# cafferychen777/flashdeconv

Measured on AMD Instinct MI355X. Metric: spots/sec to convergence (1M x 2000 x 30), higher is better.
Workload: dtype f64; 1 GPU; 1000000 spots x 2000 genes x 30 types, sketch_dim 512, k_neighbors 6, gaussian/raw family, Y float32 in HBM, tol 1e-4, max_iter 100; converged=True

## Files before the change

### flashdeconv_amd/_lib.py

```python
import ctypes
import os
import threading

import numpy as np

_HERE = os.path.dirname(os.path.abspath(__file__))
LIB_PATH = os.path.join(_HERE, "libfdx.so")

c_int = ctypes.c_int
c_i32 = ctypes.c_int32
c_i64 = ctypes.c_int64
c_double = ctypes.c_double
c_void_p = ctypes.c_void_p
c_size_t = ctypes.c_size_t
p_double = ctypes.POINTER(ctypes.c_double)
p_i64 = ctypes.POINTER(ctypes.c_int64)
p_i32 = ctypes.POINTER(ctypes.c_int32)


class FdxError(RuntimeError):
    """A libfdx call failed (message from fdx_last_error())."""


class SolveInfo(ctypes.Structure):
# ... 199 lines not shown
    "fdx_comm_init_local": (c_int, [c_void_p, c_i32, ctypes.POINTER(c_void_p)]),
    "fdx_comm_init_loopback": (c_int, [c_i32, c_i32, ctypes.POINTER(c_void_p)]),
    "fdx_comm_destroy": (c_int, [c_void_p]),
    "fdx_comm_info": (c_int, [c_void_p, p_i32, p_i32]),
    "fdx_comm_rccl_count": (c_int, [c_void_p, p_i32]),
    "fdx_comm_allreduce_sum_dev": (c_int, [c_void_p, c_void_p, c_i32, c_void_p]),
    "fdx_sharded_solve_dev": (c_int, [c_void_p, c_void_p, c_void_p, c_i64, c_void_p, c_i32, c_double, c_double, c_double, c_i32,
                                      c_void_p, c_void_p, c_i64, ctypes.POINTER(SolveInfo), p_double, p_i32, c_void_p]),
    "fdx_solver_padded_k": (c_i32, [c_i32]),
    "fdx_shard_fit_dev": (c_int, [c_void_p, c_void_p, c_void_p, c_i32, c_i64, c_i32, c_i64, p_double, c_i32, p_i32, p_double, p_double,
                                  ctypes.POINTER(ShardFitParams), c_void_p, c_void_p, p_double, ctypes.POINTER(ShardFitInfo), c_void_p]),
    "fdx_sharded_solve_padded_dev": (c_int, [c_void_p, c_void_p, c_void_p, c_i64, c_void_p, c_i32, c_i32, c_double, c_double, c_double,
                                             c_i32, c_void_p, c_void_p, c_i64, ctypes.POINTER(SolveInfo), p_double, p_i32, c_void_p]),
    "fdx_tile_schedule": (c_int, [p_i32, p_double, c_i32, c_i32, c_i32, c_i32, c_i32, p_i32, p_i32, c_void_p, p_i32, p_double,
                                  c_void_p, c_i64]),
    "fdx_sketch_path": (c_int, [c_i32, c_void_p, c_i64, c_i32, c_i32, c_i32, c_i32, p_i32, p_double, p_i32, p_i32]),
    "fdx_column_sums": (c_int, [c_void_p, c_i32, c_i64, c_i32, p_double]),
    "fdx_log1p_f32": (c_int, [c_void_p, ctypes.c_float, c_i64, c_void_p]),
    "fdx_graph_build_knn": (c_int, [p_double, c_i64, c_i32, c_i32, ctypes.POINTER(c_void_p)]),
    "fdx_graph_build_radius": (c_int, [p_double, c_i64, c_i32, c_double, ctypes.POINTER(c_void_p)]),
    "fdx_nearest_distance": (c_int, [p_double, c_i64, c_i32, p_double]),
    "fdx_graph_export_csr": (c_int, [c_void_p, p_i64, p_i32]),
    "fdx_graph_from_csr": (c_int, [p_i64, p_i64, c_i64, ctypes.POINTER(c_void_p)]),
    "fdx_graph_destroy": (c_int, [c_void_p]),
    "fdx_graph_info": (c_int, [c_void_p, p_i64, p_i64, p_i32]),
    "fdx_graph_knn_ties": (c_int, [c_void_p, p_i64]),
    "fdx_graph_knn_far": (c_int, [c_void_p, ctypes.POINTER(c_i32)]),
    "fdx_kdtree_set_threads": (c_int, [c_i32]),
    "fdx_kdtree_tune": (c_int, [c_i32, c_i64]),
    "fdx_ckdtree_indices_dev": (c_int, [c_void_p, c_i64, c_i32, p_i64, p_i32, c_void_p]),
# ... 421 lines not shown
```

### flashdeconv_amd/csrc/tile_kernels.cpp

```cpp
#include "fdx_env.h"
#include <algorithm>
#include <cmath>
#include <cstdlib>
#include <memory>
#include <mutex>

#include "fdx_internal.h"
#include "fdx_kernels.h"
#include "sketch_plan.h"
#include "tile_device.h"
#include "tile_plan.h"
#include "tile_variant.h"

namespace fdx {

struct TilePlanDevice {
    TilePlanHost h;
    DevBuf w, off, len, ent_base, slot_bucket;
    int RS = 0;
    int WB = 0;
    size_t lds = 0;
};

const double* log_table_dev(hipStream_t st) {
    static std::mutex mu;
    static double* tabs[64] = {};
    int dev = 0;
    if (hipGetDevice(&dev) != hipSuccess || dev < 0 || dev >= 64) return nullptr;
    std::lock_guard<std::mutex> lock(mu);
    if (!tabs[dev]) {
        std::vector<double> t((size_t)LOG_TAB_N);
        for (int i = 0; i < LOG_TAB_N; ++i) {
            const unsigned bits = (unsigned)(LOG_TAB_BASE + i) << LOG_TAB_SHIFT;
            float c;
// ... 23 lines not shown
}

static bool tile_cfg(int dtype, int mode, int K, int d, int logv, TileVariant* out) {
    if ((dtype != FDX_F32 && dtype != FDX_F64) || K < 1 || K > 64 || d < 1) return false;
    if (mode != FDX_PRE_RAW && mode != FDX_PRE_LOG_CPM && mode != FDX_PRE_LOG_CPM_SPARSE) return false;
    const bool raw = mode == FDX_PRE_RAW;
    TileVariant v = raw ? TileVariant{12, 4, 11} : TileVariant{16, 0, 8};
    v.TT = (K + 15) / 16;
    if (K > 32 || d > 4 * v.NWC * v.JW) {
        v = raw ? TileVariant{12, 4, 22, 4, true} : TileVariant{8, 0, 32, 4, true};
        if (d > 4 * v.NWC * v.JW) return false;
    }
    v.logv = (dtype == FDX_F32 && !raw && logv != 0) ? 2 : 0;
    v.avl2 = v.wide || (!raw && v.logv == 0);
    v.wg = v.wide && raw;
    *out = v;
    return true;
}

static size_t tile_lds_bytes(int RS, int NE, int mode, int WB = 0) {
    const size_t NEp = ((size_t)NE + 7) & ~(size_t)7;
    const size_t below = 2 * ((size_t)WB + (size_t)TILE_ROWS * RS) + NEp * (WB ? 2 : 10) + 2 * TILE_ROWS * (8 + 4);
    if (mode == FDX_PRE_RAW) return below;
    return below <= (size_t)LOG_TAB_LDS ? (size_t)160 * 1024 : (size_t)161 * 1024;
}

static const TilePlanDevice* tile_plan_for(const SketchPlan& sp, int dtype, int mode, const TileVariant& v, hipStream_t st) {
    const int sz = dtype == FDX_F32 ? 4 : 8;
    const int key = ((dtype == FDX_F32 ? 0 : 1) * 2 + (mode != FDX_PRE_RAW ? 1 : 0)) * 3 + (v.wide ? 2 : v.TT - 1);
    static_assert(SketchPlan::kTileKeys == 12, "key space of the schedules: input type x raw / log x {one tile, two tiles, wide}");
    std::lock_guard<std::mutex> lock(sp.tile_mu);
    if (sp.tile_tried[key]) return sp.tile[key].get();
    sp.tile_tried[key] = true;
    const bool dbg = fdx::env("FDX_DEBUG") != nullptr;
    if (!sp.scatter_ok || sp.host_bucket.empty()) return nullptr;
    const size_t red_bytes = tile_red_bytes(v.NWC, v.avl2, v.TT);
    const int unit = (v.wide ? 128 : 1024) / sz;
    std::unique_ptr<TilePlanDevice> best;
    int GB0 = (int)round_up(sp.G, unit);
    while ((size_t)(v.wg ? round_up((GB0 + 1) * 8, 16) : 0) + (size_t)TILE_ROWS * (GB0 * sz + TILE_ROW_PAD) < red_bytes) GB0 += unit;
    for (int GB = GB0; GB >= unit; GB -= unit) {
        const int RS = GB * sz + TILE_ROW_PAD;
        const int WB = v.wg ? (int)round_up((GB + 1) * 8, 16) : 0;
        if ((size_t)WB + (size_t)TILE_ROWS * RS < red_bytes) break;
        if (tile_lds_bytes(RS, sp.G, mode, WB) > 160 * 1024) continue;
        auto cand = std::make_unique<TilePlanDevice>();
        if (!build_tile_plan(sp.host_bucket.data(), sp.host_w.data(), sp.G, sp.d, v.NWC, v.JW, GB, &cand->h)) return nullptr;
        cand->RS = RS;
        cand->WB = WB;
        cand->lds = tile_lds_bytes(RS, cand->h.NE, mode, WB);
        if (dbg) std::fprintf(stderr, "[fdx] tile plan: G=%d d=%d waves=%d+%d GB=%d blocks=%d NE=%d steps=%d lds=%zu\n", sp.G, sp.d, v.NWC,
                              v.NWL, GB, cand->h.NBLK, cand->h.NE, cand->h.steps, cand->lds);
        if (cand->lds > 160 * 1024) continue;
        best = std::move(cand);
        break;
    }
    if (!best) return nullptr;
    TilePlanDevice& t = *best;
    auto up = [&](DevBuf& b, const void* src, size_t bytes) -> int {
        FDX_TRY(b.alloc(bytes));
        FDX_TRY(copy_h2d(b.p, src, bytes, st));
        return 0;
    };
    const int jp = JW_PAD(v.JW);
    std::vector<unsigned char> len_pad((size_t)v.NWC * t.h.NBLK * jp + 16, 0);
    for (int wv = 0; wv < v.NWC; ++wv)
        for (int c = 0; c < t.h.NBLK; ++c)
            for (int j = 0; j < v.JW; ++j)
                len_pad[((size_t)wv * t.h.NBLK + c) * jp + j] = t.h.len[((size_t)wv * t.h.NBLK + c) * v.JW + j];
    std::vector<double> wg_tab;
    if (t.WB) {
        const int per = t.WB / 8;
        wg_tab.assign((size_t)t.h.NBLK * per, 0.0);
        for (int g = 0; g < sp.G; ++g)
            if (sp.host_bucket[(size_t)g] >= 0) wg_tab[(size_t)(g / t.h.GB) * per + g % t.h.GB] = sp.host_w[(size_t)g];
        for (size_t i = 0; i < t.h.off.size(); ++i)
            if (t.h.gene[i] < 0) t.h.off[i] = (unsigned short)t.h.GB;
    }
    if ((t.WB ? up(t.w, wg_tab.data(), wg_tab.size() * 8) : up(t.w, t.h.w.data(), t.h.w.size() * 8)) ||
        up(t.off, t.h.off.data(), t.h.off.size() * 2) || up(t.len, len_pad.data(), len_pad.size()) || up(t.ent_base, t.h.ent_base.data(), t.h.ent_base.size() * 4) ||
        up(t.slot_bucket, t.h.slot_bucket.data(), t.h.slot_bucket.size() * 4))
        return nullptr;
    if (hipStreamSynchronize(st) != hipSuccess) return nullptr;
    sp.tile[key] = std::move(best);
    return sp.tile[key].get();
}

__global__ void tile_xa_kernel(const double* __restrict__ Xs, const int* __restrict__ slot_bucket, int K, int d, int n_groups,
                               int TT, double* __restrict__ XA) {
    const int i = blockIdx.x * blockDim.x + threadIdx.x;
    if (i >= n_groups * TT * 64) return;
    const int lane = i & 63, t = (i >> 6) % TT, wj = (i >> 6) / TT;
// ... 17 lines not shown
                       const SketchPlanDev& plan, const double* Xs, int K, double* H, long long ldh, double* row_sumsq,
                       hipStream_t st) {
    if (n <= 0) return 0;
    TileVariant v;
    const TilePlanDevice* t = plan.owner && tile_cfg(dtype, mode, K, d, tile_logv(), &v) ? tile_plan_for(*plan.owner, dtype, mode, v, st) : nullptr;
    if (!t) return fail(FDX_ERR_INVALID, "tile sketch: no schedule for this shape");
    const void* kern = dtype == FDX_F32 ? tile_kernel<float>(mode, v) : tile_kernel<double>(mode, v);
    if (!kern) {
        char msg[128];
        std::snprintf(msg, sizeof msg, "tile sketch: no kernel for dtype %d mode %d, waves %d + %d x %d, TT %d, AVL2 %d, LOGV %d, WG %d",
                      dtype, mode, v.NWC, v.NWL, v.JW, v.TT, (int)v.avl2, v.logv, (int)v.wg);
        return fail(FDX_ERR_INVALID, msg);
    }
    TileArgs a{};
    a.ldy = ldy; a.n = n; a.ldh = ldh; a.G = G; a.d = d; a.K = K;
    a.NE = t->h.NE; a.GB = t->h.GB; a.NBLK = t->h.NBLK; a.RS = t->RS; a.jw_used = t->h.jw_used; a.WB = t->WB;
    const double* w_tab = t->w.as<double>();
    const unsigned short* off_tab = t->off.as<unsigned short>();
    const unsigned char* len_tab = t->len.as<unsigned char>();
    const int* ent_base = t->ent_base.as<int>();
    const int* slot_bucket = t->slot_bucket.as<int>();
    const double* log_tab = nullptr;
    if (mode != FDX_PRE_RAW) {
        log_tab = log_table_dev(st);
        if (!log_tab) return fail(FDX_ERR_HIP, "tile sketch: log table upload failed");
    }
    const long long n_tiles = (n + TILE_ROWS - 1) / TILE_ROWS;
    const int grid = (int)std::min<long long>(n_tiles, 256);
    DevBuf xa;
    const double* XA = nullptr;
    if (v.avl2) {
// ... 37 lines not shown
extern "C" int fdx_log1p_f32(const float* y, float scale, int64_t n, float* out) {
    using namespace fdx;
    FDX_REQUIRE(n >= 0 && (n == 0 || (y && out)), "fdx_log1p_f32: null argument");
    if (n == 0) return 0;
    DevBuf in, res;
    FDX_TRY(in.alloc((size_t)n * 4));
    FDX_TRY(res.alloc((size_t)n * 4));
    FDX_HIP(hipMemcpy(in.p, y, (size_t)n * 4, hipMemcpyHostToDevice));
    hipLaunchKernelGGL(log1p_f32_probe_kernel, dim3((unsigned)ceil_div(n, 256)), dim3(256), 0, nullptr, in.as<float>(), scale,
                       (long long)n, res.as<float>());
    FDX_CHECK_LAUNCH();
    FDX_HIP(hipMemcpy(out, res.p, (size_t)n * 4, hipMemcpyDeviceToHost));
    return 0;
}

extern "C" int fdx_tile_schedule(const int32_t* gene_bucket, const double* gene_w, int32_t G, int32_t d, int32_t NW,
                                   int32_t JW, int32_t GB, int32_t* dims_out ,
                                   int32_t* slot_bucket_out, uint8_t* len_out, int32_t* ent_base_out, double* w_out,
                                   uint16_t* off_out, int64_t cap_entries) {
    using namespace fdx;
    FDX_REQUIRE(gene_bucket && gene_w && dims_out, "fdx_tile_schedule: null argument");
    TilePlanHost h;
    FDX_REQUIRE(build_tile_plan(gene_bucket, gene_w, G, d, NW, JW, GB, &h), "fdx_tile_schedule: shape cannot be scheduled");
    dims_out[0] = h.NBLK; dims_out[1] = h.NE; dims_out[2] = h.steps; dims_out[3] = h.max_wave_steps;
    if (!slot_bucket_out) return 0;
    FDX_REQUIRE(len_out && ent_base_out && w_out && off_out && cap_entries >= h.NE, "fdx_tile_schedule: output too small");
    std::copy(h.slot_bucket.begin(), h.slot_bucket.end(), slot_bucket_out);
    std::copy(h.len.begin(), h.len.end(), len_out);
    std::copy(h.ent_base.begin(), h.ent_base.end(), ent_base_out);
    std::copy(h.w.begin(), h.w.end(), w_out);
    std::copy(h.off.begin(), h.off.end(), off_out);
    return 0;
}

extern "C" int fdx_sketch_path(int32_t y_dtype, const void* Y_dev, int64_t ldy, int32_t G, int32_t d, int32_t K, int32_t mode_y_in,
                               const int32_t* bucket, const double* weight_y, int32_t* path_out,
                               int32_t* dims_out ) {
    using namespace fdx;
    FDX_REQUIRE(bucket && weight_y && path_out, "fdx_sketch_path: null argument");
    FDX_REQUIRE(G > 0 && K > 0 && d > 0 && ldy >= G, "fdx_sketch_path: bad shape");
    const int32_t mode_y = mode_y_in & 0xff;
    if (dims_out) std::fill(dims_out, dims_out + 6, 0);
    hipStream_t st = nullptr;
    PoolStream pool_stream(st);
    std::shared_ptr<SketchPlan> plan;
    FDX_TRY(sketch_plan_cached(bucket, weight_y, G, d, st, &plan));
    *path_out = 0;
    if (!fused_sketch_contract_ok(y_dtype, ldy, Y_dev, G, d, K, mode_y, plan->dev(), st)) return 0;
    TileVariant v;
    const TilePlanDevice* t = tile_cfg(y_dtype, mode_y, K, d, tile_logv(), &v) ? tile_plan_for(*plan, y_dtype, mode_y, v, st) : nullptr;
    FDX_REQUIRE(t != nullptr, "fdx_sketch_path: the one-kernel form was accepted without a schedule");
    *path_out = v.wide ? 2 : 1;
    if (dims_out) {
        dims_out[0] = v.NWC; dims_out[1] = v.NWL; dims_out[2] = v.JW; dims_out[3] = v.TT;
        dims_out[4] = t->h.GB; dims_out[5] = t->h.NBLK;
    }
    return 0;
}
```

### flashdeconv_amd/csrc/tile_plan.cpp

```cpp
#include "tile_plan.h"

#include <algorithm>
#include <numeric>

namespace fdx {

bool build_tile_plan(const int* gene_bucket, const double* gene_w, int G, int d, int NW, int JW, int GB, TilePlanHost* out) {
    if (G <= 0 || d <= 0 || NW <= 0 || JW <= 0 || GB <= 0 || GB > 65536) return false;
    const int n_groups = NW * JW;
    if (d > 4 * n_groups) return false;
    const int NBLK = (G + GB - 1) / GB;
    TilePlanHost& p = *out;
    p = TilePlanHost();
    p.G = G; p.d = d; p.NW = NW; p.JW = JW; p.GB = GB; p.NBLK = NBLK;

    std::vector<std::vector<int>> genes((size_t)d);
    for (int g = 0; g < G; ++g) {
        const int b = gene_bucket[g];
        if (b < 0) continue;
        if (b >= d) return false;
        genes[(size_t)b].push_back(g);
    }
    std::vector<int> cnt((size_t)d * NBLK, 0);
    for (int b = 0; b < d; ++b)
        for (int g : genes[(size_t)b]) cnt[(size_t)b * NBLK + g / GB]++;

    struct Group { int b[4]; int cost; std::vector<int> len; };
    std::vector<Group> groups((size_t)n_groups);
    std::vector<int> total((size_t)d, 0);
    for (int b = 0; b < d; ++b) total[(size_t)b] = (int)genes[(size_t)b].size();
    std::vector<char> used((size_t)d, 0);
    int n_left = d;
    for (int gi = 0; gi < n_groups; ++gi) {
        Group& gr = groups[(size_t)gi];
        gr.len.assign((size_t)NBLK, 0);
        gr.cost = 0;
        for (int q = 0; q < 4; ++q) gr.b[q] = -1;
        for (int q = 0; q < 4 && n_left > 0; ++q) {
            int best = -1, best_inc = 0;
            for (int b = 0; b < d; ++b) {
// ... 7 lines not shown
                }
            }
            used[(size_t)best] = 1;
            --n_left;
            gr.b[q] = best;
            for (int c = 0; c < NBLK; ++c) gr.len[(size_t)c] = std::max(gr.len[(size_t)c], cnt[(size_t)best * NBLK + c]);
        }
        for (int c = 0; c < NBLK; ++c) {
            if (gr.len[(size_t)c] > 255) return false;
            gr.cost += gr.len[(size_t)c];
        }
    }
    std::vector<int> gorder((size_t)n_groups);
    std::iota(gorder.begin(), gorder.end(), 0);
    std::stable_sort(gorder.begin(), gorder.end(), [&](int a, int b) { return groups[(size_t)a].cost > groups[(size_t)b].cost; });
    std::vector<std::vector<int>> of_wave((size_t)NW);
    std::vector<int> load((size_t)NW, 0);
    for (int gi : gorder) {
        int best = -1;
        for (int w = 0; w < NW; ++w)
            if ((int)of_wave[(size_t)w].size() < JW && (best < 0 || load[(size_t)w] < load[(size_t)best])) best = w;
        of_wave[(size_t)best].push_back(gi);
        load[(size_t)best] += groups[(size_t)gi].cost;
    }

    p.slot_bucket.assign((size_t)n_groups * 4, -1);
    p.len.assign((size_t)NW * NBLK * JW, 0);
    p.ent_base.assign((size_t)NW * (NBLK + 1), 0);
    p.w.clear();
    p.off.clear();
    p.gene.clear();
    for (int w = 0; w < NW; ++w) {
        int wave_steps = 0;
        for (int j = 0; j < JW; ++j)
            for (int q = 0; q < 4; ++q) {
                const int b = groups[(size_t)of_wave[(size_t)w][(size_t)j]].b[q];
                p.slot_bucket[((size_t)w * JW + j) * 4 + q] = b;
                if (b >= 0) p.jw_used = std::max(p.jw_used, j + 1);
            }
// ... 2 lines not shown
            p.ent_base[(size_t)w * (NBLK + 1) + c] = (int)p.w.size();
            for (int j = 0; j < JW; ++j) {
                const Group& gr = groups[(size_t)of_wave[(size_t)w][(size_t)j]];
                const int L = gr.len[(size_t)c];
                p.len[((size_t)w * NBLK + c) * JW + j] = (unsigned char)L;
                wave_steps += L;
                for (int t = 0; t < L; ++t)
                    for (int q = 0; q < 4; ++q) {
                        double wt = 0.0;
                        int o = 0;
                        int gid = -1;
                        const int b = gr.b[q];
                        if (b >= 0) {
                            int& k = taken[(size_t)j * 4 + q];
                            const std::vector<int>& L_b = genes[(size_t)b];
                            if (k < (int)L_b.size() && L_b[(size_t)k] / GB == c) {
                                wt = gene_w[L_b[(size_t)k]];
                                o = L_b[(size_t)k] - c * GB;
                                gid = L_b[(size_t)k];
                                ++k;
                            }
                        }
                        p.w.push_back(wt);
                        p.off.push_back((unsigned short)o);
                        p.gene.push_back(gid);
                    }
            }
        }
        p.ent_base[(size_t)w * (NBLK + 1) + NBLK] = (int)p.w.size();
        for (int q = 0; q < 8; ++q) {
            p.w.push_back(0.0);
            p.off.push_back(0);
            p.gene.push_back(-1);
// ... 15 lines not shown
```

### flashdeconv_amd/csrc/tile_plan.h

```cpp
#pragma once
#include <vector>

namespace fdx {

struct TilePlanHost {
    int G = 0, d = 0, NW = 0, JW = 0, GB = 0, NBLK = 0;
    int NE = 0;
    int steps = 0;
    int max_wave_steps = 0;
    int jw_used = 0;
    std::vector<int> slot_bucket;
    std::vector<unsigned char> len;
    std::vector<int> ent_base;
    std::vector<double> w;
    std::vector<unsigned short> off;
    std::vector<int> gene;
};

bool build_tile_plan(const int* gene_bucket, const double* gene_w, int G, int d, int NW, int JW, int GB, TilePlanHost* out);


}
```

### flashdeconv_amd/csrc/tile_sketch_kernel.h

```cpp
#pragma once
#include <type_traits>

#include "device_math.h"
#include "fdx_internal.h"
#include "tile_device.h"
#include "tile_variant.h"

namespace fdx {

template <typename T> struct TileVec;
template <> struct TileVec<float> { typedef float type __attribute__((ext_vector_type(4))); };
template <> struct TileVec<double> { typedef double type __attribute__((ext_vector_type(2))); };

__device__ __forceinline__ void dma16(const void* src, unsigned char* lds_base) {
    __builtin_amdgcn_global_load_lds((const void __attribute__((address_space(1)))*)src,
                                     (void __attribute__((address_space(3)))*)lds_base, 16, 0, 0);
}

template <typename T, int MODE, int NWC, int NWL, int JW, int TT, bool AVL2, int LOGV = 0, bool WG = false, bool FF = false>
__global__ __launch_bounds__((NWC + NWL) * 64, (NWC + NWL) / 4) void tile_sketch_kernel(
    const TileArgs a, const T* __restrict__ Yp, const int* __restrict__ row_map, const double* __restrict__ Xs,
    double* __restrict__ H, double* __restrict__ row_sumsq, const double* __restrict__ w_tab,
    const unsigned short* __restrict__ off_tab, const unsigned char* __restrict__ len_tab,
    const int* __restrict__ ent_base, const int* __restrict__ slot_bucket, const double* __restrict__ log_tab,
// ... 6 lines not shown
    constexpr int RPL = (TILE_ROWS + NWS - 1) / NWS;
    constexpr bool PAIR = tile_red_pair(NWC, AVL2);
    constexpr int NR = PAIR ? NWC / 2 : NWC;
    static_assert(!PAIR || NWC % 2 == 0, "paired reduction needs an even number of consumer waves");
    static_assert(TT == 1 || TT == 2 || TT == 4, "type tiles: 1, 2 or 4");
    constexpr int TH = tile_red_th(TT);
    constexpr int ROUNDS = TT / TH;
    constexpr int TS = TH * 4 * 64;
    static_assert(tile_red_bytes(NWC, AVL2, TT) == (size_t)NR * (TS + 64) * 8, "the host sizes the column blocks by the reduction area");
    static_assert(!FF, "the flat schedule is gone: FF only keeps the kernel's ten-parameter name");
    constexpr int NST = 2;
    const int tid = threadIdx.x, lane = tid & 63;
    const int wave = __builtin_amdgcn_readfirstlane(tid >> 6);
    const int r = lane & 15, q = lane >> 4;
    const int WB = WG ? a.WB : 0;
    const int stage_bytes = WB + TILE_ROWS * a.RS;
    const int NEp = (a.NE + 7) & ~7;
    double* w_l = reinterpret_cast<double*>(smem + (size_t)NST * stage_bytes);
    unsigned short* off_l = reinterpret_cast<unsigned short*>(w_l + (WG ? 0 : NEp));
    double* scales = reinterpret_cast<double*>(off_l + NEp);
    int* rowok = reinterpret_cast<int*>(scales + 2 * TILE_ROWS);
    double* logt = reinterpret_cast<double*>(smem + LOG_TAB_LDS);
    for (int i = tid; i < a.NE; i += NT) {
        if (!WG) w_l[i] = w_tab[i];
        off_l[i] = off_tab[i];
    }
    if (WG) {
        for (int i = tid; i < NST * TILE_ROWS * 4; i += NT)
            *reinterpret_cast<unsigned*>(smem + (size_t)(i / (TILE_ROWS * 4)) * stage_bytes + WB + ((i >> 2) % TILE_ROWS) * a.RS + a.RS - TILE_ROW_PAD + (i & 3) * 4) = 0u;
    }
    constexpr bool F32LOG = LOGV != 0 && sizeof(T) == 4 && MODE != FDX_PRE_RAW;
    if (MODE != FDX_PRE_RAW && !F32LOG)
        for (int i = tid; i < LOG_TAB_N; i += NT) logt[i] = log_tab[i];
    const long long n_tiles = (a.n + TILE_ROWS - 1) / TILE_ROWS;
    long long tile = blockIdx.x;
    if (tile >= n_tiles) return;

    const int lw = NWL > 0 ? wave - NWC : wave;
    auto load_rows = [&](long long t, const T* (&rp)[RPL]) {
#pragma unroll
        for (int k = 0; k < RPL; ++k) {
            const int rr = lw + NWS * k;
            rp[k] = nullptr;
            if (rr >= TILE_ROWS || t >= n_tiles) continue;
            const long long sp = t * TILE_ROWS + rr;
            if (sp < a.n) {
                const long long row = row_map ? (long long)row_map[sp] : sp;
                rp[k] = Yp + (size_t)row * (size_t)a.ldy;
            }
        }
    };
    auto issue_stage = [&](const T* const (&rp)[RPL], int c, int buf) {
        const int gene0 = c * a.GB;
        const int bytes = (min(a.GB, a.G - gene0)) * (int)sizeof(T);
        unsigned char* base = smem + (size_t)buf * stage_bytes + WB;
        if (WG) {
            const unsigned char* wsrc = reinterpret_cast<const unsigned char*>(w_tab) + (size_t)c * WB + lane * 16;
            for (int o = lw * 1024; o < WB; o += NWS * 1024)
                if (o + lane * 16 < WB) dma16(wsrc + o, base - WB + o);
        }
#pragma unroll
        for (int k = 0; k < RPL; ++k) {
            if (!rp[k]) continue;
            const unsigned char* src = reinterpret_cast<const unsigned char*>(rp[k] + gene0) + lane * 16;
            unsigned char* dst = base + (lw + NWS * k) * a.RS;
            for (int o = 0; o < bytes; o += 1024)
                if (o + lane * 16 < bytes) dma16(src + o, dst + o);
        }
    };
    const int nvec = a.G / PER;
    constexpr bool TWO = RPL > 1;
    auto scale_two = [&](const T* r0, const T* r1_, double* out_scale, int* out_ok, int i0, int i1) {
        const T* r1 = TWO ? r1_ : nullptr;
        const V* src0 = reinterpret_cast<const V*>(r0);
        const V* src1 = reinterpret_cast<const V*>(r1);
        double p0 = 0.0, p1 = 0.0;
        unsigned long long sg0 = 0ULL, sg1 = 0ULL;
        auto bits_of = [](T v) -> unsigned long long {
            if constexpr (sizeof(T) == 4) return (unsigned long long)__float_as_uint((float)v) << 32;
            else return (unsigned long long)__double_as_longlong((double)v);
// ... 113 lines not shown
        double acc[JW];
#pragma unroll
        for (int j = 0; j < JW; ++j) acc[j] = 0.0;
        double4_t accm[TT];
#pragma unroll
        for (int t = 0; t < TT; ++t) accm[t] = double4_t{0.0, 0.0, 0.0, 0.0};
        double sq = 0.0;
        double scale = 1.0;
        double scale_s = FDX_LOG_DOWN;
        float scale_sf = FDX_LOG_DOWN_F;
        float scale_f = 1.0f;
        bool fast = true;
        auto consume = [&](int c, auto last_tag, auto fast_tag) {
            constexpr bool LAST = decltype(last_tag)::value;
            constexpr bool FAST = decltype(fast_tag)::value;
            const unsigned char* rowb = smem + (size_t)buf * stage_bytes + WB + r * a.RS;
            const double* wgl = reinterpret_cast<const double*>(smem + (size_t)buf * stage_bytes);
            int p = ent_base[wave * (a.NBLK + 1) + c] + q;
            const unsigned long long* lens = reinterpret_cast<const unsigned long long*>(len_tab + ((size_t)wave * a.NBLK + c) * JW_PAD(JW));
            const unsigned off0 = off_l[p];
            double wv = WG ? wgl[off0] : w_l[p];
            T yv = *reinterpret_cast<const T*>(rowb + (size_t)off0 * sizeof(T));
            unsigned offn = off_l[p + 4];
            auto f = [&](T yy) -> double {
                if (MODE == FDX_PRE_RAW) return (double)yy;
                if constexpr (F32LOG) {
                    if (FAST) return (double)tile_log1p_f32((float)yy, scale_f);
                    return tile_log1p_any((double)yy * scale);
                } else {
                    if (FAST) return tile_log1p_scaled(yy, scale_s, scale_sf, lc);
                    return tile_log1p((double)yy * scale, lc);
                }
// ... 66 lines not shown
                    if ((j & 3) == 0) __builtin_amdgcn_sched_barrier(0);
#pragma unroll
                    for (int t = 0; t < TT; ++t) an[t] = *reinterpret_cast<const double*>(reinterpret_cast<const char*>(xu + (size_t)(j * TT + t) * 64) + lane8);
                }
#pragma unroll
                for (int t = 0; t < TT; ++t)
                    accm[t] = __builtin_amdgcn_mfma_f64_16x16x4f64(AVL2 ? an[t] : av[AVL2 ? 0 : j][t], acc[j], accm[t], 0, 0, 0);
                sq = fma(acc[j], acc[j], sq);
            }
        }
        par ^= 1;
        if (NWL == 0) {
#pragma unroll
            for (int k = 0; k < RPL; ++k) rowp[k] = rown[k];
        }
        double* red = reinterpret_cast<double*>(smem + (size_t)(buf ^ 1) * stage_bytes);
        double* red_sq = red + (size_t)NR * TS;
        const long long s0 = tile * TILE_ROWS;
#pragma unroll
        for (int rd = 0; rd < ROUNDS; ++rd) {
            lds_barrier();
            if (PAIR) {
                if (wave >= NR) {
#pragma unroll
                    for (int t = 0; t < TH; ++t)
#pragma unroll
                        for (int rr = 0; rr < 4; ++rr) red[(size_t)(wave - NR) * TS + (t * 4 + rr) * 64 + lane] = accm[rd * TH + t][rr];
                    if (rd == 0) red_sq[(wave - NR) * 64 + lane] = sq;
                }
                lds_barrier();
                if (wave < NR) {
// ... 19 lines not shown
                const int type = (rd * TH + (tr >> 2)) * 16 + (l >> 4) + 4 * (tr & 3);
                const long long sp = s0 + (l & 15);
                if (type < a.K && sp < a.n) H[(size_t)type * a.ldh + sp] = sum;
            }
            if (rd == 0 && row_sumsq && tid < TILE_ROWS && s0 + tid < a.n) {
                double sum = 0.0;
                for (int v = 0; v < NR; ++v)
#pragma unroll
                    for (int qq = 0; qq < 4; ++qq) sum += red_sq[v * 64 + qq * 16 + tid];
                row_sumsq[s0 + tid] = sum;
            }
        }
        if (WG) {
            lds_barrier();
            if (tid < TILE_ROWS * 4)
                *reinterpret_cast<unsigned*>(reinterpret_cast<unsigned char*>(red) + WB + (tid >> 2) * a.RS + a.RS - TILE_ROW_PAD + (tid & 3) * 4) = 0u;
        }
    }
}

}
```

### flashdeconv_amd/csrc/tile_variant.h

```cpp
#pragma once
#include <cstddef>

namespace fdx {

constexpr int TILE_ROW_PAD = 16;

struct TileArgs {
    long long ldy, n, ldh;
    int G, d, K;
    int NE, GB, NBLK, RS, jw_used;
    int WB;
};

constexpr int JW_PAD(int jw) { return (jw + 7) & ~7; }

constexpr bool tile_red_pair(int NWC, bool AVL2) { return NWC > 8 || AVL2; }
constexpr int tile_red_th(int TT) { return TT > 2 ? 2 : TT; }
constexpr size_t tile_red_bytes(int NWC, bool AVL2, int TT) {
    return (size_t)(tile_red_pair(NWC, AVL2) ? NWC / 2 : NWC) * (tile_red_th(TT) * 4 * 64 + 64) * 8;
}

struct TileVariant {
    int NWC, NWL, JW, TT;
    bool wide, avl2;
    int logv;
    bool wg;
};

template <typename T> const void* tile_kernel(int mode, const TileVariant& v);

}
```

### include/fdx.h

```cpp
#ifndef FDX_H
#define FDX_H

#include <stddef.h>
#include <stdint.h>

#ifdef __cplusplus
extern "C" {
#endif

#define FDX_OK 0
#define FDX_ERR_INVALID (-1)
#define FDX_ERR_HIP (-2)
#define FDX_ERR_UNSUPPORTED (-3)
#define FDX_ERR_INTERNAL (-4)

#define FDX_F32 0
#define FDX_F64 1

#define FDX_PRE_RAW 0
#define FDX_PRE_LOG_CPM 1
#define FDX_PRE_LOG_CPM_SPARSE 2
#define FDX_PRE_F64_MATH 0x100

int fdx_version(void);
// ... 21 lines not shown
#define FDX_SRC_U16 5
#define FDX_SRC_I32 6
#define FDX_SRC_U32 7
#define FDX_SRC_I64 8
#define FDX_SRC_U64 9
int fdx_upload_convert_dev(void* dst_dev, int32_t dst_dtype, const void* src_host, int32_t src_code, int64_t count,
                           double* max_abs_out, void* stream);
int fdx_download_dev(void* dst_host, const void* src_dev, size_t bytes, void* stream);
int fdx_pinned_copy_rate(size_t bytes, int32_t to_device, double* gbps_out);

int fdx_sketch(const void* Y, int32_t dtype, int64_t n, int32_t G, const int64_t* col_ptr, const int32_t* gene_idx,
               const double* weight, int32_t d, int32_t mode, double* Ys_out);
int fdx_tile_schedule(const int32_t* gene_bucket, const double* gene_w, int32_t G, int32_t d, int32_t NW, int32_t JW,
                      int32_t GB, int32_t* dims_out, int32_t* slot_bucket_out, uint8_t* len_out, int32_t* ent_base_out,
                      double* w_out, uint16_t* off_out, int64_t cap_entries);
int fdx_sketch_path(int32_t y_dtype, const void* Y_dev, int64_t ldy, int32_t G, int32_t d, int32_t K, int32_t mode_y,
                    const int32_t* bucket, const double* weight_y, int32_t* path_out, int32_t* dims_out);
int fdx_log1p_f32(const float* y, float scale, int64_t n, float* out);
int fdx_column_sums(const void* Y, int32_t dtype, int64_t n, int32_t G, double* sums_out);

int fdx_column_sums_dev(const void* Y_dev, int32_t dtype, int64_t n, int32_t G, int64_t ldy, double* sums_out_host,
                        void* stream);

int fdx_gene_moments_dev(const void* Y_dev, int32_t dtype, int64_t n, int32_t G, int64_t ldy, double* mean_out_host,
                         double* var_out_host, void* stream);
int fdx_gather_columns_dev(const void* Y_dev, int32_t dtype, int64_t n, int32_t G, int64_t ldy, const int32_t* idx_host,
                           int32_t G_sel, void* out_dev, void* stream);

int fdx_leverage_scores(const double* X, int32_t K, int32_t G, double regularization, double* lev_out);
typedef struct fdx_leverage_job fdx_leverage_job;
// ... 345 lines not shown
```

Before: 269.7 million spots/s.

## Use alternating unequal gene block widths and per-block wave load balancing in tile sketch

For the raw non-wide tile sketch path, the two LDS stage buffers now take alternating block widths (roughly 65/35 of a pair), so the two double-buffered stages differ in size. The tile planner also assigns bucket groups to waves by minimising the sum over blocks of the per-block maximum wave load, followed by a pairwise swap refinement, instead of balancing total cost only. The aim is to cut idle waves at each block barrier and to shape the pipeline stages better, at the cost of a more complex schedule and a slower host-side plan build. A new exported schedule API takes explicit block boundaries.

```diff
diff --git a/flashdeconv_amd/_lib.py b/flashdeconv_amd/_lib.py
--- a/flashdeconv_amd/_lib.py
+++ b/flashdeconv_amd/_lib.py
@@ -237,6 +237,8 @@
                                              c_i32, c_void_p, c_void_p, c_i64, ctypes.POINTER(SolveInfo), p_double, p_i32, c_void_p]),
     "fdx_tile_schedule": (c_int, [p_i32, p_double, c_i32, c_i32, c_i32, c_i32, c_i32, p_i32, p_i32, c_void_p, p_i32, p_double,
                                   c_void_p, c_i64]),
+    "fdx_tile_schedule_blocks": (c_int, [p_i32, p_double, c_i32, c_i32, c_i32, c_i32, p_i32, c_i32, p_i32, p_i32, c_void_p, p_i32,
+                                         p_double, c_void_p, c_i64]),
     "fdx_sketch_path": (c_int, [c_i32, c_void_p, c_i64, c_i32, c_i32, c_i32, c_i32, p_i32, p_double, p_i32, p_i32]),
     "fdx_column_sums": (c_int, [c_void_p, c_i32, c_i64, c_i32, p_double]),
     "fdx_log1p_f32": (c_int, [c_void_p, ctypes.c_float, c_i64, c_void_p]),
diff --git a/flashdeconv_amd/csrc/tile_kernels.cpp b/flashdeconv_amd/csrc/tile_kernels.cpp
--- a/flashdeconv_amd/csrc/tile_kernels.cpp
+++ b/flashdeconv_amd/csrc/tile_kernels.cpp
@@ -17,7 +17,8 @@
 struct TilePlanDevice {
     TilePlanHost h;
     DevBuf w, off, len, ent_base, slot_bucket;
-    int RS = 0;
+    int GB0 = 0, GB1 = 0;
+    int RS0 = 0, RS1 = 0;
     int WB = 0;
     size_t lds = 0;
 };
@@ -71,13 +72,25 @@
     v.logv = (dtype == FDX_F32 && !raw && logv != 0) ? 2 : 0;
     v.avl2 = v.wide || (!raw && v.logv == 0);
     v.wg = v.wide && raw;
+    v.uneven = raw && !v.wide;
     *out = v;
     return true;
 }
 
-static size_t tile_lds_bytes(int RS, int NE, int mode, int WB = 0) {
+static int tile_pair_genes(int sz, int G, int NBLK) { return (int)round_up(ceil_div(G, NBLK / 2), 64 / sz); }
+static int tile_odd_block(const TileVariant& v, int sz, int G, int NBLK, size_t red_bytes) {
+    if (!v.uneven || NBLK < 2 || NBLK % 2 != 0) return 0;
+    const int unit = 64 / sz, pair = tile_pair_genes(sz, G, NBLK);
+    const int GB1 = (int)round_up((pair * 35) / 100, unit);
+    if (GB1 <= 0 || 2 * GB1 >= pair) return 0;
+    if ((size_t)TILE_ROWS * (GB1 * sz + TILE_ROW_PAD) < red_bytes) return 0;
+    if (tile_block_gene0(NBLK - 1, pair - GB1, GB1) >= G) return 0;
+    return GB1;
+}
+
+static size_t tile_lds_bytes(int RS0, int RS1, int NE, int mode, int WB = 0) {
     const size_t NEp = ((size_t)NE + 7) & ~(size_t)7;
-    const size_t below = 2 * ((size_t)WB + (size_t)TILE_ROWS * RS) + NEp * (WB ? 2 : 10) + 2 * TILE_ROWS * (8 + 4);
+    const size_t below = 2 * (size_t)WB + (size_t)TILE_ROWS * ((size_t)RS0 + RS1) + NEp * (WB ? 2 : 10) + 2 * TILE_ROWS * (8 + 4);
     if (mode == FDX_PRE_RAW) return below;
     return below <= (size_t)LOG_TAB_LDS ? (size_t)160 * 1024 : (size_t)161 * 1024;
 }
@@ -100,12 +113,13 @@
         const int RS = GB * sz + TILE_ROW_PAD;
         const int WB = v.wg ? (int)round_up((GB + 1) * 8, 16) : 0;
         if ((size_t)WB + (size_t)TILE_ROWS * RS < red_bytes) break;
-        if (tile_lds_bytes(RS, sp.G, mode, WB) > 160 * 1024) continue;
+        if (tile_lds_bytes(RS, RS, sp.G, mode, WB) > 160 * 1024) continue;
         auto cand = std::make_unique<TilePlanDevice>();
         if (!build_tile_plan(sp.host_bucket.data(), sp.host_w.data(), sp.G, sp.d, v.NWC, v.JW, GB, &cand->h)) return nullptr;
-        cand->RS = RS;
+        cand->GB0 = cand->GB1 = GB;
+        cand->RS0 = cand->RS1 = RS;
         cand->WB = WB;
-        cand->lds = tile_lds_bytes(RS, cand->h.NE, mode, WB);
+        cand->lds = tile_lds_bytes(RS, RS, cand->h.NE, mode, WB);
         if (dbg) std::fprintf(stderr, "[fdx] tile plan: G=%d d=%d waves=%d+%d GB=%d blocks=%d NE=%d steps=%d lds=%zu\n", sp.G, sp.d, v.NWC,
                               v.NWL, GB, cand->h.NBLK, cand->h.NE, cand->h.steps, cand->lds);
         if (cand->lds > 160 * 1024) continue;
@@ -113,6 +127,21 @@
         break;
     }
     if (!best) return nullptr;
+    if (const int GB1 = tile_odd_block(v, sz, sp.G, best->h.NBLK, red_bytes)) {
+        const int NBLK = best->h.NBLK, GB0 = tile_pair_genes(sz, sp.G, NBLK) - GB1;
+        std::vector<int> blk((size_t)NBLK + 1, sp.G);
+        for (int c = 0; c < NBLK; ++c) blk[(size_t)c] = tile_block_gene0(c, GB0, GB1);
+        auto cand = std::make_unique<TilePlanDevice>();
+        if (!build_tile_plan(sp.host_bucket.data(), sp.host_w.data(), sp.G, sp.d, v.NWC, v.JW, blk.data(), NBLK, &cand->h)) return nullptr;
+        cand->GB0 = GB0;
+        cand->GB1 = GB1;
+        cand->RS0 = GB0 * sz + TILE_ROW_PAD;
+        cand->RS1 = GB1 * sz + TILE_ROW_PAD;
+        cand->lds = tile_lds_bytes(cand->RS0, cand->RS1, cand->h.NE, mode);
+        if (dbg) std::fprintf(stderr, "[fdx] tile plan: G=%d d=%d unequal blocks %d / %d x %d NE=%d steps=%d block_max=%d lds=%zu\n", sp.G, sp.d, GB0,
+                              GB1, NBLK, cand->h.NE, cand->h.steps, cand->h.block_max_steps, cand->lds);
+        if (cand->lds <= 160 * 1024 && (size_t)TILE_ROWS * cand->RS1 >= red_bytes) best = std::move(cand);
+    }
     TilePlanDevice& t = *best;
     auto up = [&](DevBuf& b, const void* src, size_t bytes) -> int {
         FDX_TRY(b.alloc(bytes));
@@ -130,9 +159,9 @@
         const int per = t.WB / 8;
         wg_tab.assign((size_t)t.h.NBLK * per, 0.0);
         for (int g = 0; g < sp.G; ++g)
-            if (sp.host_bucket[(size_t)g] >= 0) wg_tab[(size_t)(g / t.h.GB) * per + g % t.h.GB] = sp.host_w[(size_t)g];
+            if (sp.host_bucket[(size_t)g] >= 0) wg_tab[(size_t)(g / t.GB0) * per + g % t.GB0] = sp.host_w[(size_t)g];
         for (size_t i = 0; i < t.h.off.size(); ++i)
-            if (t.h.gene[i] < 0) t.h.off[i] = (unsigned short)t.h.GB;
+            if (t.h.gene[i] < 0) t.h.off[i] = (unsigned short)t.GB0;
     }
     if ((t.WB ? up(t.w, wg_tab.data(), wg_tab.size() * 8) : up(t.w, t.h.w.data(), t.h.w.size() * 8)) ||
         up(t.off, t.h.off.data(), t.h.off.size() * 2) || up(t.len, len_pad.data(), len_pad.size()) || up(t.ent_base, t.h.ent_base.data(), t.h.ent_base.size() * 4) ||
@@ -180,7 +209,9 @@
     }
     TileArgs a{};
     a.ldy = ldy; a.n = n; a.ldh = ldh; a.G = G; a.d = d; a.K = K;
-    a.NE = t->h.NE; a.GB = t->h.GB; a.NBLK = t->h.NBLK; a.RS = t->RS; a.jw_used = t->h.jw_used; a.WB = t->WB;
+    a.NE = t->h.NE; a.GB0 = t->GB0; a.GB1 = t->GB1; a.NBLK = t->h.NBLK; a.RS0 = t->RS0; a.RS1 = t->RS1; a.jw_used = t->h.jw_used; a.WB = t->WB;
+    a.SB1 = t->WB + TILE_ROWS * t->RS0;
+    a.ST = a.SB1 + t->WB + TILE_ROWS * t->RS1;
     const double* w_tab = t->w.as<double>();
     const unsigned short* off_tab = t->off.as<unsigned short>();
     const unsigned char* len_tab = t->len.as<unsigned char>();
@@ -248,15 +279,11 @@
     return 0;
 }
 
-extern "C" int fdx_tile_schedule(const int32_t* gene_bucket, const double* gene_w, int32_t G, int32_t d, int32_t NW,
-                                   int32_t JW, int32_t GB, int32_t* dims_out ,
-                                   int32_t* slot_bucket_out, uint8_t* len_out, int32_t* ent_base_out, double* w_out,
-                                   uint16_t* off_out, int64_t cap_entries) {
-    using namespace fdx;
-    FDX_REQUIRE(gene_bucket && gene_w && dims_out, "fdx_tile_schedule: null argument");
-    TilePlanHost h;
-    FDX_REQUIRE(build_tile_plan(gene_bucket, gene_w, G, d, NW, JW, GB, &h), "fdx_tile_schedule: shape cannot be scheduled");
-    dims_out[0] = h.NBLK; dims_out[1] = h.NE; dims_out[2] = h.steps; dims_out[3] = h.max_wave_steps;
+static int tile_schedule_out(const fdx::TilePlanHost& h, int n_dims, int32_t* dims_out, int32_t* slot_bucket_out, uint8_t* len_out,
+                             int32_t* ent_base_out, double* w_out, uint16_t* off_out, int64_t cap_entries) {
+    using namespace fdx;
+    const int32_t dims[5] = {h.NBLK, h.NE, h.steps, h.max_wave_steps, h.block_max_steps};
+    std::copy(dims, dims + n_dims, dims_out);
     if (!slot_bucket_out) return 0;
     FDX_REQUIRE(len_out && ent_base_out && w_out && off_out && cap_entries >= h.NE, "fdx_tile_schedule: output too small");
     std::copy(h.slot_bucket.begin(), h.slot_bucket.end(), slot_bucket_out);
@@ -265,6 +292,29 @@
     std::copy(h.w.begin(), h.w.end(), w_out);
     std::copy(h.off.begin(), h.off.end(), off_out);
     return 0;
+}
+
+extern "C" int fdx_tile_schedule(const int32_t* gene_bucket, const double* gene_w, int32_t G, int32_t d, int32_t NW,
+                                   int32_t JW, int32_t GB, int32_t* dims_out ,
+                                   int32_t* slot_bucket_out, uint8_t* len_out, int32_t* ent_base_out, double* w_out,
+                                   uint16_t* off_out, int64_t cap_entries) {
+    using namespace fdx;
+    FDX_REQUIRE(gene_bucket && gene_w && dims_out, "fdx_tile_schedule: null argument");
+    TilePlanHost h;
+    FDX_REQUIRE(build_tile_plan(gene_bucket, gene_w, G, d, NW, JW, GB, &h), "fdx_tile_schedule: shape cannot be scheduled");
+    return tile_schedule_out(h, 4, dims_out, slot_bucket_out, len_out, ent_base_out, w_out, off_out, cap_entries);
+}
+
+extern "C" int fdx_tile_schedule_blocks(const int32_t* gene_bucket, const double* gene_w, int32_t G, int32_t d, int32_t NW,
+                                          int32_t JW, const int32_t* blk_start, int32_t n_blocks,
+                                          int32_t* dims_out ,
+                                          int32_t* slot_bucket_out, uint8_t* len_out, int32_t* ent_base_out, double* w_out,
+                                          uint16_t* off_out, int64_t cap_entries) {
+    using namespace fdx;
+    FDX_REQUIRE(gene_bucket && gene_w && blk_start && dims_out, "fdx_tile_schedule_blocks: null argument");
+    TilePlanHost h;
+    FDX_REQUIRE(build_tile_plan(gene_bucket, gene_w, G, d, NW, JW, blk_start, n_blocks, &h), "fdx_tile_schedule_blocks: shape cannot be scheduled");
+    return tile_schedule_out(h, 5, dims_out, slot_bucket_out, len_out, ent_base_out, w_out, off_out, cap_entries);
 }
 
 extern "C" int fdx_sketch_path(int32_t y_dtype, const void* Y_dev, int64_t ldy, int32_t G, int32_t d, int32_t K, int32_t mode_y_in,
@@ -287,7 +337,7 @@
     *path_out = v.wide ? 2 : 1;
     if (dims_out) {
         dims_out[0] = v.NWC; dims_out[1] = v.NWL; dims_out[2] = v.JW; dims_out[3] = v.TT;
-        dims_out[4] = t->h.GB; dims_out[5] = t->h.NBLK;
+        dims_out[4] = t->GB0; dims_out[5] = t->h.NBLK;
     }
     return 0;
 }
diff --git a/flashdeconv_amd/csrc/tile_plan.cpp b/flashdeconv_amd/csrc/tile_plan.cpp
--- a/flashdeconv_amd/csrc/tile_plan.cpp
+++ b/flashdeconv_amd/csrc/tile_plan.cpp
@@ -6,13 +6,30 @@
 namespace fdx {
 
 bool build_tile_plan(const int* gene_bucket, const double* gene_w, int G, int d, int NW, int JW, int GB, TilePlanHost* out) {
-    if (G <= 0 || d <= 0 || NW <= 0 || JW <= 0 || GB <= 0 || GB > 65536) return false;
+    if (G <= 0 || GB <= 0 || GB > 65536) return false;
+    std::vector<int> blk;
+    for (int g = 0; g < G; g += GB) blk.push_back(g);
+    const int NBLK = (int)blk.size();
+    blk.push_back(G);
+    return build_tile_plan(gene_bucket, gene_w, G, d, NW, JW, blk.data(), NBLK, out);
+}
+
+bool build_tile_plan(const int* gene_bucket, const double* gene_w, int G, int d, int NW, int JW, const int* blk_start, int NBLK,
+                     TilePlanHost* out) {
+    if (G <= 0 || d <= 0 || NW <= 0 || JW <= 0 || NBLK <= 0 || !blk_start || blk_start[0] != 0 || blk_start[NBLK] != G) return false;
     const int n_groups = NW * JW;
     if (d > 4 * n_groups) return false;
-    const int NBLK = (G + GB - 1) / GB;
     TilePlanHost& p = *out;
     p = TilePlanHost();
-    p.G = G; p.d = d; p.NW = NW; p.JW = JW; p.GB = GB; p.NBLK = NBLK;
+    p.G = G; p.d = d; p.NW = NW; p.JW = JW; p.NBLK = NBLK;
+    p.blk.assign(blk_start, blk_start + NBLK + 1);
+    std::vector<int> block_of((size_t)G);
+    for (int c = 0; c < NBLK; ++c) {
+        const int width = p.blk[(size_t)c + 1] - p.blk[(size_t)c];
+        if (width <= 0 || width > 65536) return false;
+        p.GB = std::max(p.GB, width);
+        for (int g = p.blk[(size_t)c]; g < p.blk[(size_t)c + 1]; ++g) block_of[(size_t)g] = c;
+    }
 
     std::vector<std::vector<int>> genes((size_t)d);
     for (int g = 0; g < G; ++g) {
@@ -23,7 +40,7 @@
     }
     std::vector<int> cnt((size_t)d * NBLK, 0);
     for (int b = 0; b < d; ++b)
-        for (int g : genes[(size_t)b]) cnt[(size_t)b * NBLK + g / GB]++;
+        for (int g : genes[(size_t)b]) cnt[(size_t)b * NBLK + block_of[(size_t)g]]++;
 
     struct Group { int b[4]; int cost; std::vector<int> len; };
     std::vector<Group> groups((size_t)n_groups);
@@ -61,15 +78,61 @@
     std::vector<int> gorder((size_t)n_groups);
     std::iota(gorder.begin(), gorder.end(), 0);
     std::stable_sort(gorder.begin(), gorder.end(), [&](int a, int b) { return groups[(size_t)a].cost > groups[(size_t)b].cost; });
-    std::vector<std::vector<int>> of_wave((size_t)NW);
-    std::vector<int> load((size_t)NW, 0);
+    std::vector<int> wave_of((size_t)n_groups, -1), n_of((size_t)NW, 0);
+    std::vector<int> load((size_t)NW * NBLK, 0);
+    struct Score { long long f, sq; bool operator<(const Score& o) const { return f < o.f || (f == o.f && sq < o.sq); } };
+    auto score = [&]() {
+        Score s{0, 0};
+        for (int c = 0; c < NBLK; ++c) {
+            int mx = 0;
+            for (int w = 0; w < NW; ++w) {
+                const int l = load[(size_t)w * NBLK + c];
+                mx = std::max(mx, l);
+                s.sq += (long long)l * l;
+            }
+            s.f += mx;
+        }
+        return s;
+    };
+    auto move = [&](int gi, int w, int sign) {
+        for (int c = 0; c < NBLK; ++c) load[(size_t)w * NBLK + c] += sign * groups[(size_t)gi].len[(size_t)c];
+    };
     for (int gi : gorder) {
         int best = -1;
-        for (int w = 0; w < NW; ++w)
-            if ((int)of_wave[(size_t)w].size() < JW && (best < 0 || load[(size_t)w] < load[(size_t)best])) best = w;
-        of_wave[(size_t)best].push_back(gi);
-        load[(size_t)best] += groups[(size_t)gi].cost;
+        Score best_s{0, 0};
+        for (int w = 0; w < NW; ++w) {
+            if (n_of[(size_t)w] >= JW) continue;
+            move(gi, w, +1);
+            const Score s = score();
+            move(gi, w, -1);
+            if (best < 0 || s < best_s) { best = w; best_s = s; }
+        }
+        move(gi, best, +1);
+        wave_of[(size_t)gi] = best;
+        ++n_of[(size_t)best];
     }
+    Score cur = score();
+    for (int pass = 0, improved = 1; improved && pass < 64; ++pass) {
+        improved = 0;
+        for (int a = 0; a < n_groups; ++a)
+            for (int b = a + 1; b < n_groups; ++b) {
+                const int wa = wave_of[(size_t)a], wb = wave_of[(size_t)b];
+                if (wa == wb || groups[(size_t)a].len == groups[(size_t)b].len) continue;
+                move(a, wa, -1); move(b, wb, -1); move(a, wb, +1); move(b, wa, +1);
+                const Score s = score();
+                if (s < cur) {
+                    cur = s;
+                    wave_of[(size_t)a] = wb;
+                    wave_of[(size_t)b] = wa;
+                    improved = 1;
+                } else {
+                    move(a, wb, -1); move(b, wa, -1); move(a, wa, +1); move(b, wb, +1);
+                }
+            }
+    }
+    p.block_max_steps = (int)cur.f;
+    std::vector<std::vector<int>> of_wave((size_t)NW);
+    for (int gi : gorder) of_wave[(size_t)wave_of[(size_t)gi]].push_back(gi);
 
     p.slot_bucket.assign((size_t)n_groups * 4, -1);
     p.len.assign((size_t)NW * NBLK * JW, 0);
@@ -102,9 +165,9 @@
                         if (b >= 0) {
                             int& k = taken[(size_t)j * 4 + q];
                             const std::vector<int>& L_b = genes[(size_t)b];
-                            if (k < (int)L_b.size() && L_b[(size_t)k] / GB == c) {
+                            if (k < (int)L_b.size() && block_of[(size_t)L_b[(size_t)k]] == c) {
                                 wt = gene_w[L_b[(size_t)k]];
-                                o = L_b[(size_t)k] - c * GB;
+                                o = L_b[(size_t)k] - p.blk[(size_t)c];
                                 gid = L_b[(size_t)k];
                                 ++k;
                             }
diff --git a/flashdeconv_amd/csrc/tile_plan.h b/flashdeconv_amd/csrc/tile_plan.h
--- a/flashdeconv_amd/csrc/tile_plan.h
+++ b/flashdeconv_amd/csrc/tile_plan.h
@@ -8,7 +8,9 @@
     int NE = 0;
     int steps = 0;
     int max_wave_steps = 0;
+    int block_max_steps = 0;
     int jw_used = 0;
+    std::vector<int> blk;
     std::vector<int> slot_bucket;
     std::vector<unsigned char> len;
     std::vector<int> ent_base;
@@ -17,6 +19,8 @@
     std::vector<int> gene;
 };
 
+bool build_tile_plan(const int* gene_bucket, const double* gene_w, int G, int d, int NW, int JW, const int* blk_start, int NBLK,
+                     TilePlanHost* out);
 bool build_tile_plan(const int* gene_bucket, const double* gene_w, int G, int d, int NW, int JW, int GB, TilePlanHost* out);
 
 
diff --git a/flashdeconv_amd/csrc/tile_sketch_kernel.h b/flashdeconv_amd/csrc/tile_sketch_kernel.h
--- a/flashdeconv_amd/csrc/tile_sketch_kernel.h
+++ b/flashdeconv_amd/csrc/tile_sketch_kernel.h
@@ -44,9 +44,10 @@
     const int wave = __builtin_amdgcn_readfirstlane(tid >> 6);
     const int r = lane & 15, q = lane >> 4;
     const int WB = WG ? a.WB : 0;
-    const int stage_bytes = WB + TILE_ROWS * a.RS;
+    auto buf_base = [&](int b) { return b ? a.SB1 : 0; };
+    auto buf_rs = [&](int b) { return b ? a.RS1 : a.RS0; };
     const int NEp = (a.NE + 7) & ~7;
-    double* w_l = reinterpret_cast<double*>(smem + (size_t)NST * stage_bytes);
+    double* w_l = reinterpret_cast<double*>(smem + (size_t)a.ST);
     unsigned short* off_l = reinterpret_cast<unsigned short*>(w_l + (WG ? 0 : NEp));
     double* scales = reinterpret_cast<double*>(off_l + NEp);
     int* rowok = reinterpret_cast<int*>(scales + 2 * TILE_ROWS);
@@ -56,8 +57,10 @@
         off_l[i] = off_tab[i];
     }
     if (WG) {
-        for (int i = tid; i < NST * TILE_ROWS * 4; i += NT)
-            *reinterpret_cast<unsigned*>(smem + (size_t)(i / (TILE_ROWS * 4)) * stage_bytes + WB + ((i >> 2) % TILE_ROWS) * a.RS + a.RS - TILE_ROW_PAD + (i & 3) * 4) = 0u;
+        for (int i = tid; i < NST * TILE_ROWS * 4; i += NT) {
+            const int b = i / (TILE_ROWS * 4);
+            *reinterpret_cast<unsigned*>(smem + (size_t)buf_base(b) + WB + ((i >> 2) % TILE_ROWS) * buf_rs(b) + buf_rs(b) - TILE_ROW_PAD + (i & 3) * 4) = 0u;
+        }
     }
     constexpr bool F32LOG = LOGV != 0 && sizeof(T) == 4 && MODE != FDX_PRE_RAW;
     if (MODE != FDX_PRE_RAW && !F32LOG)
@@ -81,9 +84,10 @@
         }
     };
     auto issue_stage = [&](const T* const (&rp)[RPL], int c, int buf) {
-        const int gene0 = c * a.GB;
-        const int bytes = (min(a.GB, a.G - gene0)) * (int)sizeof(T);
-        unsigned char* base = smem + (size_t)buf * stage_bytes + WB;
+        const int gene0 = tile_block_gene0(c, a.GB0, a.GB1);
+        const int bytes = (min(tile_block_width(c, a.GB0, a.GB1), a.G - gene0)) * (int)sizeof(T);
+        unsigned char* base = smem + (size_t)buf_base(buf) + WB;
+        const int RS = buf_rs(buf);
         if (WG) {
             const unsigned char* wsrc = reinterpret_cast<const unsigned char*>(w_tab) + (size_t)c * WB + lane * 16;
             for (int o = lw * 1024; o < WB; o += NWS * 1024)
@@ -93,7 +97,7 @@
         for (int k = 0; k < RPL; ++k) {
             if (!rp[k]) continue;
             const unsigned char* src = reinterpret_cast<const unsigned char*>(rp[k] + gene0) + lane * 16;
-            unsigned char* dst = base + (lw + NWS * k) * a.RS;
+            unsigned char* dst = base + (lw + NWS * k) * RS;
             for (int o = 0; o < bytes; o += 1024)
                 if (o + lane * 16 < bytes) dma16(src + o, dst + o);
         }
@@ -237,8 +241,8 @@
         auto consume = [&](int c, auto last_tag, auto fast_tag) {
             constexpr bool LAST = decltype(last_tag)::value;
             constexpr bool FAST = decltype(fast_tag)::value;
-            const unsigned char* rowb = smem + (size_t)buf * stage_bytes + WB + r * a.RS;
-            const double* wgl = reinterpret_cast<const double*>(smem + (size_t)buf * stage_bytes);
+            const unsigned char* rowb = smem + (size_t)buf_base(buf) + WB + r * buf_rs(buf);
+            const double* wgl = reinterpret_cast<const double*>(smem + (size_t)buf_base(buf));
             int p = ent_base[wave * (a.NBLK + 1) + c] + q;
             const unsigned long long* lens = reinterpret_cast<const unsigned long long*>(len_tab + ((size_t)wave * a.NBLK + c) * JW_PAD(JW));
             const unsigned off0 = off_l[p];
@@ -335,7 +339,7 @@
 #pragma unroll
             for (int k = 0; k < RPL; ++k) rowp[k] = rown[k];
         }
-        double* red = reinterpret_cast<double*>(smem + (size_t)(buf ^ 1) * stage_bytes);
+        double* red = reinterpret_cast<double*>(smem + (size_t)buf_base(buf ^ 1));
         double* red_sq = red + (size_t)NR * TS;
         const long long s0 = tile * TILE_ROWS;
 #pragma unroll
@@ -385,7 +389,7 @@
         if (WG) {
             lds_barrier();
             if (tid < TILE_ROWS * 4)
-                *reinterpret_cast<unsigned*>(reinterpret_cast<unsigned char*>(red) + WB + (tid >> 2) * a.RS + a.RS - TILE_ROW_PAD + (tid & 3) * 4) = 0u;
+                *reinterpret_cast<unsigned*>(reinterpret_cast<unsigned char*>(red) + WB + (tid >> 2) * buf_rs(buf ^ 1) + buf_rs(buf ^ 1) - TILE_ROW_PAD + (tid & 3) * 4) = 0u;
         }
     }
 }
diff --git a/flashdeconv_amd/csrc/tile_variant.h b/flashdeconv_amd/csrc/tile_variant.h
--- a/flashdeconv_amd/csrc/tile_variant.h
+++ b/flashdeconv_amd/csrc/tile_variant.h
@@ -8,9 +8,12 @@
 struct TileArgs {
     long long ldy, n, ldh;
     int G, d, K;
-    int NE, GB, NBLK, RS, jw_used;
+    int NE, GB0, GB1, NBLK, RS0, RS1, SB1, ST, jw_used;
     int WB;
 };
+
+constexpr int tile_block_gene0(int c, int GB0, int GB1) { return (c >> 1) * (GB0 + GB1) + (c & 1) * GB0; }
+constexpr int tile_block_width(int c, int GB0, int GB1) { return (c & 1) ? GB1 : GB0; }
 
 constexpr int JW_PAD(int jw) { return (jw + 7) & ~7; }
 
@@ -25,6 +28,7 @@
     bool wide, avl2;
     int logv;
     bool wg;
+    bool uneven;
 };
 
 template <typename T> const void* tile_kernel(int mode, const TileVariant& v);
diff --git a/include/fdx.h b/include/fdx.h
--- a/include/fdx.h
+++ b/include/fdx.h
@@ -59,6 +59,9 @@
 int fdx_tile_schedule(const int32_t* gene_bucket, const double* gene_w, int32_t G, int32_t d, int32_t NW, int32_t JW,
                       int32_t GB, int32_t* dims_out, int32_t* slot_bucket_out, uint8_t* len_out, int32_t* ent_base_out,
                       double* w_out, uint16_t* off_out, int64_t cap_entries);
+int fdx_tile_schedule_blocks(const int32_t* gene_bucket, const double* gene_w, int32_t G, int32_t d, int32_t NW, int32_t JW,
+                             const int32_t* blk_start, int32_t n_blocks, int32_t* dims_out, int32_t* slot_bucket_out,
+                             uint8_t* len_out, int32_t* ent_base_out, double* w_out, uint16_t* off_out, int64_t cap_entries);
 int fdx_sketch_path(int32_t y_dtype, const void* Y_dev, int64_t ldy, int32_t G, int32_t d, int32_t K, int32_t mode_y,
                     const int32_t* bucket, const double* weight_y, int32_t* path_out, int32_t* dims_out);
 int fdx_log1p_f32(const float* y, float scale, int64_t n, float* out);
```

Result: faster. 274.7 million spots/s, median of 5 (+1.9%).
